# superlinear-ai/raglite

Measured on NVIDIA H100. Metric: queries/sec multi-vector MaxSim over 10M chunks, higher is better.
Workload: dtype f32

## Files before the change

### raglite_b200/csrc/hopper_ptx.cuh

```cuda
#pragma once
#include <cuda.h>
#include <cuda_runtime.h>
#include <stdint.h>

namespace rl {
namespace tc {

__device__ __forceinline__ uint32_t smem_u32(const void* p) { return (uint32_t)__cvta_generic_to_shared(p); }

__device__ __forceinline__ void mbar_init(uint64_t* bar, uint32_t count) {
  asm volatile("mbarrier.init.shared::cta.b64 [%0], %1;" ::"r"(smem_u32(bar)), "r"(count) : "memory");
}
__device__ __forceinline__ void mbar_arrive(uint64_t* bar) {
  asm volatile("mbarrier.arrive.shared::cta.b64 _, [%0];" ::"r"(smem_u32(bar)) : "memory");
}
__device__ __forceinline__ void mbar_arrive_expect_tx(uint64_t* bar, uint32_t bytes) {
  asm volatile("mbarrier.arrive.expect_tx.shared::cta.b64 _, [%0], %1;" ::"r"(smem_u32(bar)), "r"(bytes) : "memory");
}
__device__ __forceinline__ bool mbar_try_wait(uint64_t* bar, uint32_t parity) {
  uint32_t ok;
  asm volatile(
      "{\n\t.reg .pred p;\n\t"
      "mbarrier.try_wait.parity.shared::cta.b64 p, [%1], %2;\n\t"
      "selp.u32 %0, 1, 0, p;\n\t}"
      : "=r"(ok)
      : "r"(smem_u32(bar)), "r"(parity)
      : "memory");
  return ok != 0;
}
__device__ __forceinline__ void mbar_wait(uint64_t* bar, uint32_t parity) {
  if (mbar_try_wait(bar, parity)) return;
  const long long t0 = clock64();
  while (!mbar_try_wait(bar, parity)) {
    if (clock64() - t0 > 20000000000ll) __trap();
  }
}
__device__ __forceinline__ void fence_barrier_init() { asm volatile("fence.mbarrier_init.release.cluster;" ::: "memory"); }
__device__ __forceinline__ void fence_proxy_async() { asm volatile("fence.proxy.async.shared::cta;" ::: "memory"); }

__device__ __forceinline__ void bulk_g2s(void* smem_dst, const void* gsrc, uint32_t bytes, uint64_t* bar) {
  asm volatile("cp.async.bulk.shared::cluster.global.mbarrier::complete_tx::bytes [%0], [%1], %2, [%3];" ::"r"(
                   smem_u32(smem_dst)),
               "l"(gsrc), "r"(bytes), "r"(smem_u32(bar))
               : "memory");
}
__device__ __forceinline__ void tma_load_2d(void* smem_dst, const CUtensorMap* tmap, int c0, int c1, uint64_t* bar) {
  asm volatile(
      "cp.async.bulk.tensor.2d.shared::cluster.global.tile.mbarrier::complete_tx::bytes [%0], [%1, {%3, %4}], [%2];"
      ::"r"(smem_u32(smem_dst)), "l"(tmap), "r"(smem_u32(bar)), "r"(c0), "r"(c1)
      : "memory");
}
__device__ __forceinline__ void tma_prefetch_2d(const CUtensorMap* tmap, int c0, int c1) {
  asm volatile("cp.async.bulk.prefetch.tensor.2d.L2.global.tile [%0, {%1, %2}];" ::"l"(tmap), "r"(c0), "r"(c1) : "memory");
}

__device__ __forceinline__ void prefetch_l2(const void* p) { asm volatile("prefetch.global.L2 [%0];" ::"l"(p)); }
__device__ __forceinline__ float4 ldg_stream(const float* p) {
  float4 v;
  asm volatile("ld.global.nc.L1::no_allocate.v4.f32 {%0, %1, %2, %3}, [%4];"
               : "=f"(v.x), "=f"(v.y), "=f"(v.z), "=f"(v.w)
               : "l"(p));
  return v;
}
__device__ __forceinline__ uint4 ldg_stream_u4(const void* p) {
  uint4 v;
  asm volatile("ld.global.nc.L1::no_allocate.v4.u32 {%0, %1, %2, %3}, [%4];"
               : "=r"(v.x), "=r"(v.y), "=r"(v.z), "=r"(v.w)
               : "l"(p));
  return v;
}

__device__ __forceinline__ void named_bar_sync(int id, int count) {
  asm volatile("bar.sync %0, %1;" ::"r"(id), "r"(count) : "memory");
}

__device__ __forceinline__ uint64_t make_kmajor_sw128_desc(uint32_t smem_addr) {
  return (uint64_t)((smem_addr >> 4) & 0x3FFFu) | (1ull << 16) | (64ull << 32) | (1ull << 62);
}
__device__ __forceinline__ void wgmma_fence() { asm volatile("wgmma.fence.sync.aligned;" ::: "memory"); }
__device__ __forceinline__ void wgmma_commit() { asm volatile("wgmma.commit_group.sync.aligned;" ::: "memory"); }
template <int N>
__device__ __forceinline__ void wgmma_wait() { asm volatile("wgmma.wait_group.sync.aligned %0;" ::"n"(N) : "memory"); }

__device__ __forceinline__ void wgmma_m64n128k16(float (&d)[64], uint64_t a_desc, uint64_t b_desc, uint32_t accumulate) {
  asm volatile(
      "{\n\t.reg .pred p;\n\t"
      "setp.ne.b32 p, %66, 0;\n\t"
      "wgmma.mma_async.sync.aligned.m64n128k16.f32.f16.f16 "
      "{%0, %1, %2, %3, %4, %5, %6, %7, %8, %9, %10, %11, %12, %13, %14, %15, "
      "%16, %17, %18, %19, %20, %21, %22, %23, %24, %25, %26, %27, %28, %29, %30, %31, "
      "%32, %33, %34, %35, %36, %37, %38, %39, %40, %41, %42, %43, %44, %45, %46, %47, "
      "%48, %49, %50, %51, %52, %53, %54, %55, %56, %57, %58, %59, %60, %61, %62, %63}, "
      "%64, %65, p, 1, 1, 0, 0;\n\t}"
      : "+f"(d[0]), "+f"(d[1]), "+f"(d[2]), "+f"(d[3]), "+f"(d[4]), "+f"(d[5]), "+f"(d[6]), "+f"(d[7]),
        "+f"(d[8]), "+f"(d[9]), "+f"(d[10]), "+f"(d[11]), "+f"(d[12]), "+f"(d[13]), "+f"(d[14]), "+f"(d[15]),
        "+f"(d[16]), "+f"(d[17]), "+f"(d[18]), "+f"(d[19]), "+f"(d[20]), "+f"(d[21]), "+f"(d[22]), "+f"(d[23]),
        "+f"(d[24]), "+f"(d[25]), "+f"(d[26]), "+f"(d[27]), "+f"(d[28]), "+f"(d[29]), "+f"(d[30]), "+f"(d[31]),
        "+f"(d[32]), "+f"(d[33]), "+f"(d[34]), "+f"(d[35]), "+f"(d[36]), "+f"(d[37]), "+f"(d[38]), "+f"(d[39]),
        "+f"(d[40]), "+f"(d[41]), "+f"(d[42]), "+f"(d[43]), "+f"(d[44]), "+f"(d[45]), "+f"(d[46]), "+f"(d[47]),
        "+f"(d[48]), "+f"(d[49]), "+f"(d[50]), "+f"(d[51]), "+f"(d[52]), "+f"(d[53]), "+f"(d[54]), "+f"(d[55]),
        "+f"(d[56]), "+f"(d[57]), "+f"(d[58]), "+f"(d[59]), "+f"(d[60]), "+f"(d[61]), "+f"(d[62]), "+f"(d[63])
      : "l"(a_desc), "l"(b_desc), "r"(accumulate)
      : "memory");
}
template <int NACC>
__device__ __forceinline__ void wgmma_slice(float (&d)[NACC], uint64_t a_desc, uint64_t b_desc, bool accumulate) {
  static_assert(NACC == 64 || NACC == 128, "wgmma_slice: N is 128 or 256");
#pragma unroll
  for (int k = 0; k < 4; ++k) {
    const uint32_t acc = (accumulate || k > 0) ? 1u : 0u;
    float(&lo)[64] = *reinterpret_cast<float(*)[64]>(&d[0]);
    wgmma_m64n128k16(lo, a_desc + (uint64_t)(2 * k), b_desc + (uint64_t)(2 * k), acc);
    if constexpr (NACC == 128) {
      float(&hi)[64] = *reinterpret_cast<float(*)[64]>(&d[64]);
      wgmma_m64n128k16(hi, a_desc + (uint64_t)(2 * k), b_desc + (uint64_t)(2 * k + (128 * 128 >> 4)), acc);
    }
  }
}

template <int R>
__device__ __forceinline__ void setmaxnreg_dec() { asm volatile("setmaxnreg.dec.sync.aligned.u32 %0;" ::"n"(R)); }
template <int R>
__device__ __forceinline__ void setmaxnreg_inc() { asm volatile("setmaxnreg.inc.sync.aligned.u32 %0;" ::"n"(R)); }

}
}
```

### raglite_b200/csrc/scan_wgmma.cu

```cuda
#include <cuda.h>
#include <cuda_fp16.h>

#include <cstdlib>
#include <cstring>
#include <type_traits>

#include "hopper_ptx.cuh"
#include "scan_wgmma.cuh"

namespace rl {

namespace {

using namespace tc;

constexpr int kTileM = 128;
constexpr int kSliceK = 64;
constexpr int kNumConsumerWarps = 8;
constexpr int kNumConsumers = kNumConsumerWarps * 32;
constexpr int kFirstLoaderWarp = 8;
constexpr int kNumLoaderWarps = 8;
constexpr int kThreads = (kFirstLoaderWarp + kNumLoaderWarps) * 32;
constexpr int kLoaderRegs = 72;
constexpr int kConsumerRegs = 184;
static_assert(kLoaderRegs + kConsumerRegs == 2 * 65536 / kThreads, "the register split must use exactly the CTA's registers");
constexpr int kMaxStages = 8;
constexpr int kABytes = kTileM * 128;
constexpr uint32_t kSmemBudget = 227 * 1024;
template <int NQ>
__host__ __device__ constexpr int prefetch_items() { return NQ == 128 ? 6 : 0; }
constexpr int kListCap = 1024;
constexpr int kFlushFirst = 192;
constexpr int kFlushAt = 512;
constexpr int kRefreshEvery = 16;
constexpr int kMaxBatchPerLaunch = 1024;

inline int query_group_width(const rl_scan_params* p) {
  const int n_ks = (p->d + kSliceK - 1) / kSliceK;
  return (p->B > 128 && p->e_dtype != 1 && n_ks >= 16) ? 256 : 128;
}

struct TcArgs {
  ScanArgs a;
  const __half* qimg;
  const float* q_scale;
  const float* row_stats;
  int nq;
  int nq_last;
  int par_groups;
  int n_ks;
  int stages;
  int pf_pairs;
};

__device__ __forceinline__ float pow2_scale(float max_abs) {
  return max_abs > 0.f ? exp2f(-ceilf(log2f(max_abs))) : 1.f;
}

struct SmemLayout {
  uint64_t* full;
  uint64_t* empty;
  float* thr;
  float* cs;
  float* thr0;
  float* inv_w;
  uint32_t* hist;
  int* cnt;
  int* basev;
  int* list_n;
  uint32_t* list;
  unsigned char* stage_base;
};

template <int NQ>
__host__ __device__ constexpr uint32_t stage_bytes() { return kABytes + NQ * 128u; }
template <int NQ>
__host__ __device__ constexpr uint32_t tail_bytes() {
  return 2 * kMaxStages * 8 + NQ * (6u * 4u + (uint32_t)kHistBins * 2u) + 16 + kListCap * 12;
}

template <int METRIC, bool EF16, int NQ>
__global__ void __launch_bounds__(kThreads, 1) scan_wgmma_kernel(const __grid_constant__ CUtensorMap tmE, const TcArgs t) {
  extern __shared__ unsigned char smem_dyn[];
  const int P = t.par_groups > 1 ? t.par_groups : 1;
  const int pg = P > 1 ? (int)(blockIdx.x % (unsigned)P) : 0;
  ScanArgs a = t.a;
  const float* q_scale_g = t.q_scale;
  const __half* qimg_g = t.qimg;
  const int nq = (pg == P - 1) ? t.nq_last : t.nq;
  if (P > 1) {
    const int q0p = pg * NQ;
    a.B = min(NQ, t.a.B - q0p);
    a.thr += q0p; a.cand_cnt += q0p; a.eps += q0p; a.hist_inv_w += q0p; a.q_inv_norm += q0p;
    if (a.cnt_all != nullptr) a.cnt_all += q0p;
    a.dump += (size_t)q0p * a.n_sample_rows;
    a.cand += (size_t)q0p * a.cap;
    a.ghist += (size_t)q0p * kHistBins;
    q_scale_g += q0p;
    qimg_g += (size_t)pg * t.n_ks * NQ * kSliceK;
  }
  constexpr uint32_t sbytes = stage_bytes<NQ>();
  SmemLayout s;
  s.full = reinterpret_cast<uint64_t*>(smem_dyn);
  s.empty = s.full + kMaxStages;
  s.thr = reinterpret_cast<float*>(s.empty + kMaxStages);
  s.cs = s.thr + NQ;
  s.thr0 = s.cs + NQ;
  s.inv_w = s.thr0 + NQ;
  s.hist = reinterpret_cast<uint32_t*>(s.inv_w + NQ);
  s.cnt = reinterpret_cast<int*>(s.hist + NQ * kHistBins / 2);
  s.basev = s.cnt + NQ;
  s.list_n = s.basev + NQ;
  s.list = reinterpret_cast<uint32_t*>(s.list_n + 4);
  unsigned char* tail_end = smem_dyn + tail_bytes<NQ>();
  s.stage_base = tail_end + ((1024u - (smem_u32(tail_end) & 1023u)) & 1023u);

  const int warp = threadIdx.x >> 5, lane = threadIdx.x & 31;
  const uint32_t n_tiles = (uint32_t)a.n_mode_blocks;
  const uint32_t first = blockIdx.x / (uint32_t)P;
  const uint32_t stride = gridDim.x / (uint32_t)P;
  const int64_t my_tiles = first < n_tiles ? (n_tiles - first + stride - 1) / stride : 0;
  auto ord_of = [&](int64_t tile) -> uint32_t { return first + (uint32_t)tile * stride; };
  auto block_of = [&](uint32_t ord) -> int64_t {
    const uint32_t S = (uint32_t)a.S;
    return a.dump_mode ? ord * S : (S <= 1u ? ord : ord + ord / (S - 1u) + 1u);
  };
  const uint32_t qbytes = (uint32_t)nq * 128u;
  const unsigned char* qsrc = reinterpret_cast<const unsigned char*>(qimg_g);
  const bool q_thread = threadIdx.x == kFirstLoaderWarp * 32;
  auto put_query = [&](int stage, int ks) {
    mbar_arrive_expect_tx(&s.full[stage], qbytes);
    bulk_g2s(s.stage_base + (size_t)stage * sbytes + kABytes, qsrc + (size_t)ks * qbytes, qbytes, &s.full[stage]);
  };

  if (threadIdx.x == 0) {
    for (int i = 0; i < t.stages; ++i) {
      mbar_init(&s.full[i], (EF16 ? 0 : kNumLoaderWarps) + 1);
      mbar_init(&s.empty[i], kNumConsumerWarps);
    }
    fence_barrier_init();
  }
  for (int i = threadIdx.x; i < NQ; i += blockDim.x) {
    s.thr[i] = (i < a.B && !a.dump_mode) ? a.thr[i] : __int_as_float(0x7f800000);
    s.cs[i] = (i < a.B) ? q_scale_g[i] : 0.f;
    s.cnt[i] = 0;
    s.thr0[i] = s.thr[i];
    s.inv_w[i] = (i < a.B && !a.dump_mode) ? a.hist_inv_w[i] : 0.f;
  }
  for (int i = threadIdx.x; i < NQ * kHistBins / 2; i += blockDim.x) s.hist[i] = 0u;
  if (threadIdx.x == 0) { s.list_n[0] = 0; s.list_n[1] = 0; }
  __syncthreads();
  auto cos_noscale_of = [&]() -> bool {
    return METRIC == RL_METRIC_COSINE &&
           (EF16 || (t.row_stats[2] > 0.f && t.row_stats[2] <= 2.f && t.row_stats[1] <= 1024.f &&
                     t.row_stats[3] == 0.f));
  };

  const bool fast_f32 = !EF16 && a.d % kSliceK == 0 && (t.n_ks & 1) == 0 && a.ld * 64 < (int64_t(1) << 32) &&
                        (METRIC != RL_METRIC_COSINE || cos_noscale_of());
  if (EF16 && warp >= kFirstLoaderWarp) {
    if constexpr (NQ == 256) setmaxnreg_dec<kLoaderRegs>();
    if (q_thread) {
      const int64_t total_items = my_tiles * t.n_ks;
      int ks = 0, stage = 0;
      uint32_t phase = 0;
      int64_t tile = 0;
      auto tile_row0 = [&](int64_t v) -> int { return v < my_tiles ? (int)(block_of(ord_of(v)) * kTileM) : -1; };
      int row0 = tile_row0(0), row0_next = tile_row0(1);
      for (int64_t item = 0; item < total_items; ++item) {
        mbar_wait(&s.empty[stage], phase ^ 1u);
        mbar_arrive_expect_tx(&s.full[stage], qbytes + (uint32_t)kABytes);
        tma_load_2d(s.stage_base + (size_t)stage * sbytes, &tmE, ks * kSliceK, row0, &s.full[stage]);
        bulk_g2s(s.stage_base + (size_t)stage * sbytes + kABytes, qsrc + (size_t)ks * qbytes, qbytes, &s.full[stage]);
        if (row0_next >= 0 && pg == 0) tma_prefetch_2d(&tmE, ks * kSliceK, row0_next);
        if (++ks == t.n_ks) { ks = 0; ++tile; row0 = row0_next; row0_next = tile_row0(tile + 1); }
        if (++stage == t.stages) { stage = 0; phase ^= 1u; }
      }
    }
  } else if (warp >= kFirstLoaderWarp && fast_f32) {
    if constexpr (NQ == 256) setmaxnreg_dec<kLoaderRegs>();
    const int lt = threadIdx.x - kFirstLoaderWarp * 32;
    const int c4 = lt & 15;
    const int r0 = lt >> 4;
    const float gscale = (METRIC == RL_METRIC_COSINE) ? 1.f : pow2_scale(t.row_stats[1]);
    const bool mul = gscale != 1.f;
    uint32_t n_ks = (uint32_t)t.n_ks, n_stages = (uint32_t)t.stages;
    uint32_t pitch16 = (uint32_t)(a.ld * 16 * (int64_t)sizeof(float));
    uint32_t sw_off = (uint32_t)r0 * 128u + ((((uint32_t)c4 >> 1) ^ ((uint32_t)r0 & 7u)) << 4) + (((uint32_t)c4 & 1u) << 3);
    asm volatile("" : "+r"(n_ks), "+r"(n_stages), "+r"(pitch16), "+r"(sw_off));
    const uint32_t total_items = (uint32_t)my_tiles * n_ks;

    struct Cursor { int64_t tile; uint32_t ks; int rows; const unsigned char* ptr; };
    Cursor ld{0, 0u, 0, nullptr};
    auto ld_set_tile = [&]() {
      ld.rows = 0;
      if (ld.tile < my_tiles) {
        const int64_t blk = block_of(ord_of(ld.tile));
        const int64_t rem = a.n_rows - blk * kTileM;
        ld.rows = rem < kTileM ? (int)rem : kTileM;
        ld.ptr = reinterpret_cast<const unsigned char*>(a.E + (size_t)(blk * kTileM + r0) * a.ld + c4 * 4);
      }
    };
    Cursor pf{0, 0u, 0, nullptr};
    auto pf_set_tile = [&]() {
      pf.rows = 0;
      if (pg == 0 && t.pf_pairs > 0 && pf.tile < my_tiles) {
        const int64_t blk = block_of(ord_of(pf.tile));
        const int64_t rem = a.n_rows - blk * kTileM;
        pf.rows = rem < kTileM ? (int)rem : kTileM;
        pf.ptr = reinterpret_cast<const unsigned char*>(a.E + (size_t)(blk * kTileM + (lt >> 1)) * a.ld + (lt & 1) * 32);
        if (METRIC == RL_METRIC_COSINE && lt < 4 && lt * 32 < pf.rows) prefetch_l2(a.inv_norm + blk * kTileM + lt * 32);
      }
    };
    auto pf_pair = [&]() {
      if ((lt >> 1) < pf.rows) { prefetch_l2(pf.ptr); prefetch_l2(pf.ptr + 256); }
      pf.ptr += 512;
      pf.ks += 2;
      if (pf.ks == n_ks) { pf.ks = 0; ++pf.tile; pf_set_tile(); }
    };
    float4 ringA[8], ringB[8];
    auto issue = [&](float4 (&buf)[8], int rows, const unsigned char* src) {
      if (rows == kTileM) {
#pragma unroll
        for (int i = 0; i < 8; ++i) buf[i] = ldg_stream(reinterpret_cast<const float*>(src + (size_t)((uint32_t)i * pitch16)));
      } else {
#pragma unroll
        for (int i = 0; i < 8; ++i) {
          if (r0 + 16 * i < rows) buf[i] = ldg_stream(reinterpret_cast<const float*>(src + (size_t)((uint32_t)i * pitch16)));
          else buf[i] = make_float4(0.f, 0.f, 0.f, 0.f);
        }
      }
    };
    uint32_t stage = 0, phase = 0, st_ks = 0;
    unsigned char* a_dst = s.stage_base + sw_off;
    auto store = [&](const float4 (&buf)[8]) {
      mbar_wait(&s.empty[stage], phase ^ 1u);
      if (q_thread) put_query((int)stage, (int)st_ks);
      if (++st_ks == n_ks) st_ks = 0;
#pragma unroll
      for (int i = 0; i < 8; ++i) {
        float4 v = buf[i];
        if (mul) { v.x *= gscale; v.y *= gscale; v.z *= gscale; v.w *= gscale; }
        const __half2 h01 = __floats2half2_rn(v.x, v.y);
        const __half2 h23 = __floats2half2_rn(v.z, v.w);
        uint2 packed;
        packed.x = *reinterpret_cast<const uint32_t*>(&h01);
        packed.y = *reinterpret_cast<const uint32_t*>(&h23);
        *reinterpret_cast<uint2*>(a_dst + i * 16 * 128) = packed;
      }
      __syncwarp();
      if (lane == 0) mbar_arrive(&s.full[stage]);
      a_dst += sbytes;
      if (++stage == n_stages) { stage = 0; phase ^= 1u; a_dst = s.stage_base + sw_off; }
    };

    ld_set_tile();
    pf_set_tile();
    for (int i = 0; i < t.pf_pairs + 1; ++i) pf_pair();
    if constexpr (NQ == 128) {
      issue(ringA, ld.rows, ld.ptr);
      issue(ringB, ld.rows, ld.ptr + 256);
      for (uint32_t item = 0; item < total_items; item += 2) {
        ld.ptr += 512;
        ld.ks += 2;
        if (ld.ks == n_ks) { ld.ks = 0; ++ld.tile; ld_set_tile(); }
        const int rows = ld.rows;
        const unsigned char* src = ld.ptr;
        store(ringA);
        issue(ringA, rows, src);
        store(ringB);
        issue(ringB, rows, src + 256);
        pf_pair();
      }
    } else {
      issue(ringA, ld.rows, ld.ptr);
      for (uint32_t item = 0; item < total_items; item += 2) {
        const int rows = ld.rows;
        const unsigned char* src = ld.ptr;
        ld.ptr += 512;
        ld.ks += 2;
        if (ld.ks == n_ks) { ld.ks = 0; ++ld.tile; ld_set_tile(); }
        store(ringA);
        issue(ringA, rows, src + 256);
        store(ringA);
        issue(ringA, ld.rows, ld.ptr);
        if constexpr (prefetch_items<NQ>() > 0) pf_pair();
      }
    }
  } else if (warp >= kFirstLoaderWarp) {
    if constexpr (NQ == 256) setmaxnreg_dec<kLoaderRegs>();
    const int lt = threadIdx.x - kFirstLoaderWarp * 32;
    const int c4 = lt & 15;
    const int r0 = lt >> 4;
    const float gscale = (METRIC == RL_METRIC_COSINE) ? 1.f : pow2_scale(t.row_stats[1]);
    const bool noscale = (METRIC == RL_METRIC_COSINE) ? cos_noscale_of() : (gscale == 1.f);
    const uint32_t total_items = (uint32_t)my_tiles * (uint32_t)t.n_ks;
    constexpr int kInFlight = NQ == 128 ? 2 : 1;
    float4 ring[kInFlight][8];
    float rs[8];

    const size_t pitch16_bytes = (size_t)a.ld * 16 * sizeof(float);
    const size_t slice_bytes = kSliceK * sizeof(float);
    int64_t ld_tile = 0;
    int ld_ks = 0, ld_rows = 0;
    const unsigned char* ld_ptr = nullptr;
    auto ld_set_tile = [&]() {
      if (ld_tile < my_tiles) {
        const int64_t blk = block_of(ord_of(ld_tile));
        const int64_t rem = a.n_rows - blk * kTileM;
        ld_rows = rem < kTileM ? (int)rem : kTileM;
        ld_ptr = reinterpret_cast<const unsigned char*>(a.E + (size_t)(blk * kTileM + r0) * a.ld + c4 * 4);
      } else {
        ld_rows = 0;
      }
    };
    int64_t pf_tile = 0;
    int pf_ks = 0, pf_rows = 0;
    const unsigned char* pf_ptr = nullptr;
    auto pf_set_tile = [&]() {
      if (pg == 0 && pf_tile < my_tiles) {
        const int64_t blk = block_of(ord_of(pf_tile));
        const int64_t rem = a.n_rows - blk * kTileM;
        pf_rows = rem < kTileM ? (int)rem : kTileM;
        pf_ptr = reinterpret_cast<const unsigned char*>(a.E + (size_t)(blk * kTileM + (lt >> 1)) * a.ld + (lt & 1) * 32);
        if (METRIC == RL_METRIC_COSINE && lt < 4 && lt * 32 < pf_rows) prefetch_l2(a.inv_norm + blk * kTileM + lt * 32);
      } else {
        pf_rows = 0;
      }
    };
    auto prefetch_item = [&]() {
      if ((lt >> 1) < pf_rows && pf_ks * kSliceK + (lt & 1) * 32 < a.d) prefetch_l2(pf_ptr);
      pf_ptr += slice_bytes;
      if (++pf_ks == t.n_ks) {
        pf_ks = 0;
        ++pf_tile;
        pf_set_tile();
      }
    };
    auto issue_item = [&](float4 (&buf)[8]) {
      const bool col_ok = ld_ks * kSliceK + c4 * 4 < a.d;
      const int rows_left = ld_rows - r0;
      const unsigned char* p = ld_ptr;
      if (col_ok && ld_rows == kTileM) {
#pragma unroll
        for (int i = 0; i < 8; ++i) {
          buf[i] = ldg_stream(reinterpret_cast<const float*>(p));
          p += pitch16_bytes;
        }
      } else {
#pragma unroll
        for (int i = 0; i < 8; ++i) {
          if (col_ok && 16 * i < rows_left) buf[i] = ldg_stream(reinterpret_cast<const float*>(p));
          else buf[i] = make_float4(0.f, 0.f, 0.f, 0.f);
          p += pitch16_bytes;
        }
      }
      ld_ptr += slice_bytes;
      if (++ld_ks == t.n_ks) {
        ld_ks = 0;
        ++ld_tile;
        ld_set_tile();
      }
      if constexpr (prefetch_items<NQ>() > 0) prefetch_item();
    };

    int64_t st_tile = 0;
    int st_ks = 0, stage = 0;
    uint32_t phase = 0;
    auto fetch_scales = [&](int64_t tile) {
#pragma unroll
      for (int i = 0; i < 8; ++i) rs[i] = (METRIC == RL_METRIC_COSINE) ? 0.f : gscale;
      if (METRIC == RL_METRIC_COSINE && !noscale && tile < my_tiles) {
        const int64_t row0 = block_of(ord_of(tile)) * kTileM + r0;
        const int64_t rows_left = a.n_rows - row0;
#pragma unroll
        for (int i = 0; i < 8; ++i) {
          if (16 * i < rows_left) rs[i] = __ldg(a.inv_norm + row0 + 16 * i);
        }
      }
    };
    const uint32_t sw_off = (uint32_t)r0 * 128u + ((((uint32_t)c4 >> 1) ^ ((uint32_t)r0 & 7u)) << 4) + (((uint32_t)c4 & 1u) << 3);
    auto process = [&](float4 (&buf)[8]) {
      mbar_wait(&s.empty[stage], phase ^ 1u);
      if (q_thread) put_query(stage, st_ks);
      unsigned char* A = s.stage_base + (size_t)stage * sbytes + sw_off;
      if (noscale) {
#pragma unroll
        for (int i = 0; i < 8; ++i) {
          const __half2 h01 = __floats2half2_rn(buf[i].x, buf[i].y);
          const __half2 h23 = __floats2half2_rn(buf[i].z, buf[i].w);
          uint2 packed;
          packed.x = *reinterpret_cast<const uint32_t*>(&h01);
          packed.y = *reinterpret_cast<const uint32_t*>(&h23);
          *reinterpret_cast<uint2*>(A + i * 16 * 128) = packed;
        }
      } else {
#pragma unroll
        for (int i = 0; i < 8; ++i) {
          const __half2 h01 = __floats2half2_rn(buf[i].x * rs[i], buf[i].y * rs[i]);
          const __half2 h23 = __floats2half2_rn(buf[i].z * rs[i], buf[i].w * rs[i]);
          uint2 packed;
          packed.x = *reinterpret_cast<const uint32_t*>(&h01);
          packed.y = *reinterpret_cast<const uint32_t*>(&h23);
          *reinterpret_cast<uint2*>(A + i * 16 * 128) = packed;
        }
      }
      __syncwarp();
      if (lane == 0) mbar_arrive(&s.full[stage]);
      issue_item(buf);
      if (++stage == t.stages) { stage = 0; phase ^= 1u; }
      if (++st_ks == t.n_ks) { st_ks = 0; ++st_tile; fetch_scales(st_tile); }
    };

    fetch_scales(0);
    ld_set_tile();
    pf_set_tile();
    for (int i = 0; i < prefetch_items<NQ>(); ++i) prefetch_item();
    for (int i = 0; i < kInFlight; ++i) issue_item(ring[i]);
    for (uint32_t item = 0; item < total_items; item += kInFlight) {
      process(ring[0]);
      if constexpr (kInFlight == 2) {
        if (item + 1 < total_items) process(ring[1]);
      }
    }
  } else {
    if constexpr (NQ == 256) setmaxnreg_inc<kConsumerRegs>();
    const int wg = warp >> 2;
    const int r_lo = wg * 64 + (warp & 3) * 16 + (lane >> 2);
    const int c_lane = 2 * (lane & 3);
    const int et = threadIdx.x;
    bool flushed_once = false;
    int stage = 0;
    uint32_t phase = 0;
    float acc[NQ / 2];
    const bool cos_noscale = cos_noscale_of();
    for (int64_t tile = 0; tile < my_tiles; ++tile) {
      int prev = -1;
      for (int ks = 0; ks < t.n_ks; ++ks) {
        mbar_wait(&s.full[stage], phase);
        fence_proxy_async();
        const uint32_t st_addr = smem_u32(s.stage_base + (size_t)stage * sbytes);
        wgmma_fence();
        wgmma_slice(acc, make_kmajor_sw128_desc(st_addr + (uint32_t)wg * (64u * 128u)), make_kmajor_sw128_desc(st_addr + kABytes),
                    ks > 0);
        wgmma_commit();
        if (prev >= 0) {
          wgmma_wait<1>();
          __syncwarp();
          if (lane == 0) mbar_arrive(&s.empty[prev]);
        }
        prev = stage;
        if (++stage == t.stages) { stage = 0; phase ^= 1u; }
      }
      wgmma_wait<0>();
      __syncwarp();
      if (lane == 0) mbar_arrive(&s.empty[prev]);

      const int64_t ord = ord_of(tile);
      const int64_t blk = block_of(ord);
      int r_in[2];
      int64_t row[2];
      bool valid[2], masked_alive[2];
      float bias[2], lane_scale[2];
#pragma unroll
      for (int h = 0; h < 2; ++h) {
        r_in[h] = r_lo + 8 * h;
        row[h] = blk * kTileM + r_in[h];
        valid[h] = row[h] < a.n_rows;
        masked_alive[h] = false;
        if (valid[h] && a.row_allowed != nullptr) {
          valid[h] = a.row_allowed[row[h]] != 0;
          if (!valid[h] && a.cnt_all != nullptr) masked_alive[h] = a.row_alive == nullptr || a.row_alive[row[h]] != 0;
        }
        bias[h] = (METRIC == RL_METRIC_L2 && valid[h]) ? -a.sq_norm[row[h]] : 0.f;
        lane_scale[h] = (METRIC == RL_METRIC_COSINE && cos_noscale && valid[h]) ? __ldg(a.inv_norm + row[h]) : 1.f;
      }
      auto key_of = [&](float accv, int h, float cs) -> float {
        return METRIC != RL_METRIC_COSINE ? fmaf(accv, cs, bias[h]) : accv * lane_scale[h];
      };
      if (a.dump_mode) {
#pragma unroll
        for (int c8 = 0; c8 < NQ / 8; ++c8) {
#pragma unroll
          for (int e = 0; e < 4; ++e) {
            const int h = e >> 1, col = 8 * c8 + c_lane + (e & 1);
            if (col < a.B) {
              const float key = key_of(acc[4 * c8 + e], h, s.cs[col]);
              a.dump[(size_t)col * a.n_sample_rows + ord * kTileM + r_in[h]] = valid[h] ? key : kNegInf;
            }
          }
        }
      } else {
#pragma unroll
        for (int c8 = 0; c8 < NQ / 8; ++c8) {
          if (8 * c8 >= nq) break;
          const int c = 8 * c8 + c_lane;
          const float2 th = *reinterpret_cast<const float2*>(s.thr + c);
          const float2 sc = METRIC != RL_METRIC_COSINE ? *reinterpret_cast<const float2*>(s.cs + c) : make_float2(0.f, 0.f);
#pragma unroll
          for (int e = 0; e < 4; ++e) {
            const int h = e >> 1, col = c + (e & 1);
            const float key = key_of(acc[4 * c8 + e], h, (e & 1) ? sc.y : sc.x);
            if (key >= ((e & 1) ? th.y : th.x)) {
              if (masked_alive[h]) atomicAdd(a.cnt_all + col, 1);
              if (valid[h]) {
                const int pos = atomicAdd(&s.list_n[0], 1);
                const int hb = col * kHistBins + hist_bin(key, s.thr0[col], s.inv_w[col]);
                atomicAdd(&s.hist[hb >> 1], 1u << ((hb & 1) * 16));
                if (pos < kListCap) {
                  s.list[pos * 3 + 0] = (uint32_t)col;
                  s.list[pos * 3 + 1] = __float_as_uint(key);
                  s.list[pos * 3 + 2] = (uint32_t)row[h];
                } else {
                  emit_candidate(a, col, key, (int32_t)row[h]);
                }
              }
            }
          }
        }
        named_bar_sync(1, kNumConsumers);
        const int n_all = s.list_n[0];
        named_bar_sync(1, kNumConsumers);
        const bool last = tile + 1 == my_tiles;
        const bool do_flush = n_all >= (flushed_once ? kFlushAt : kFlushFirst) || (last && n_all > 0);
        if (do_flush) {
          flushed_once = true;
          const int n = min(n_all, kListCap);
          for (int e = et; e < n; e += kNumConsumers) {
            const int col = (int)s.list[e * 3 + 0];
            s.list[e * 3 + 0] = (uint32_t)col | ((uint32_t)atomicAdd(&s.cnt[col], 1) << 16);
          }
          named_bar_sync(1, kNumConsumers);
          for (int col = et; col < NQ; col += kNumConsumers) {
            const int c = s.cnt[col];
            if (c > 0) {
              s.basev[col] = atomicAdd(a.cand_cnt + col, c);
              s.cnt[col] = 0;
            }
          }
          for (int w = et; w < NQ * kHistBins / 2; w += kNumConsumers) {
            const uint32_t h = s.hist[w];
            if (h != 0u) {
              if (h & 0xFFFFu) atomicAdd(a.ghist + 2 * w, (int)(h & 0xFFFFu));
              if (h >> 16) atomicAdd(a.ghist + 2 * w + 1, (int)(h >> 16));
              s.hist[w] = 0u;
            }
          }
          named_bar_sync(1, kNumConsumers);
          if (et == 0) s.list_n[0] = 0;
          for (int e = et; e < n; e += kNumConsumers) {
            const uint32_t w0 = s.list[e * 3 + 0];
            const int col = (int)(w0 & 0xFFFFu);
            const int slot = s.basev[col] + (int)(w0 >> 16);
            if (slot < a.cap)
              a.cand[(size_t)col * a.cap + slot] = Cand{__uint_as_float(s.list[e * 3 + 1]), (int32_t)s.list[e * 3 + 2]};
          }
        }
        const bool periodic = (tile % kRefreshEvery) == kRefreshEvery - 1;
        if ((do_flush || periodic) && !last) {
          for (int col = et; col < a.B; col += kNumConsumers) {
            const int4* gh = reinterpret_cast<const int4*>(a.ghist + (size_t)col * kHistBins);
            int cnts[kHistBins];
#pragma unroll
            for (int q4 = 0; q4 < kHistBins / 4; ++q4) {
              const int4 v4 = __ldcg(gh + q4);
              cnts[4 * q4] = v4.x; cnts[4 * q4 + 1] = v4.y; cnts[4 * q4 + 2] = v4.z; cnts[4 * q4 + 3] = v4.w;
            }
            int cum = 0, best = -1;
#pragma unroll
            for (int bb = kHistBins - 1; bb >= 1; --bb) {
              cum += cnts[bb];
              if (best < 0 && cum >= a.sel_count) best = bb;
            }
            if (best >= 1 && s.inv_w[col] > 0.f) {
              const float nt = s.thr0[col] + (float)best / s.inv_w[col] - 2.f * a.eps[col];
              if (nt > s.thr[col]) s.thr[col] = nt;
            }
          }
        }
        if (do_flush || periodic) named_bar_sync(1, kNumConsumers);
      }
    }
  }
}

__global__ void __launch_bounds__(128) query_image_kernel(const float* __restrict__ Q, int B, int d, int metric,
                                                          const float* __restrict__ q_inv_norm,
                                                          const float* __restrict__ row_stats, float* __restrict__ q_scale,
                                                          __half* __restrict__ qimg, int n_ks, int rows_scaled, int gw) {
  __shared__ float red[4];
  const int b = blockIdx.x;
  const int group = b / gw, n = b % gw;
  const int nq = min(gw, (B - group * gw + 15) / 16 * 16);
  const float* q = Q + (size_t)b * d;
  float scale;
  if (metric == RL_METRIC_COSINE) {
    scale = q_inv_norm[b];
    if (threadIdx.x == 0) q_scale[b] = 1.f;
  } else {
    float m = 0.f;
    for (int c = threadIdx.x; c < d; c += blockDim.x) m = fmaxf(m, fabsf(q[c]));
#pragma unroll
    for (int o = 16; o > 0; o >>= 1) m = fmaxf(m, __shfl_xor_sync(0xffffffffu, m, o));
    if ((threadIdx.x & 31) == 0) red[threadIdx.x >> 5] = m;
    __syncthreads();
    m = fmaxf(fmaxf(red[0], red[1]), fmaxf(red[2], red[3]));
    scale = pow2_scale(m);
    const float rs_e = rows_scaled ? pow2_scale(row_stats[1]) : 1.f;
    if (threadIdx.x == 0) q_scale[b] = (metric == RL_METRIC_L2 ? 2.f : 1.f) / (scale * rs_e);
  }
  __half* img = qimg + (size_t)group * n_ks * gw * kSliceK;
  for (int c = threadIdx.x; c < n_ks * kSliceK; c += blockDim.x) {
    const int ks = c / kSliceK, e = c % kSliceK;
    const float v = c < d ? q[c] * scale : 0.f;
    const int chunk = e >> 3, within = e & 7;
    const size_t off = ((size_t)ks * nq + n) * kSliceK + (size_t)(((chunk ^ (n & 7)) << 3) + within);
    img[off] = __float2half_rn(v);
  }
}

typedef CUresult (*ScanEncodeTiledFn)(CUtensorMap*, CUtensorMapDataType, cuuint32_t, void*, const cuuint64_t*, const cuuint64_t*,
                                      const cuuint32_t*, const cuuint32_t*, CUtensorMapInterleave, CUtensorMapSwizzle,
                                      CUtensorMapL2promotion, CUtensorMapFloatOOBfill);
ScanEncodeTiledFn scan_encode_tiled_fn() {
  static ScanEncodeTiledFn fn = []() -> ScanEncodeTiledFn {
    void* p = nullptr;
    cudaDriverEntryPointQueryResult q;
    if (cudaGetDriverEntryPoint("cuTensorMapEncodeTiled", &p, cudaEnableDefault, &q) != cudaSuccess || q != cudaDriverEntryPointSuccess)
      return nullptr;
    return reinterpret_cast<ScanEncodeTiledFn>(p);
  }();
  return fn;
}
bool make_corpus_tensor_map(CUtensorMap* tm, const void* E, int64_t n_rows, int64_t ld, int d) {
  ScanEncodeTiledFn enc = scan_encode_tiled_fn();
  if (enc == nullptr || (reinterpret_cast<uintptr_t>(E) & 15) != 0 || (ld * 2) % 16 != 0 || n_rows >= (int64_t(1) << 31)) return false;
  const cuuint64_t gdim[2] = {(cuuint64_t)d, (cuuint64_t)n_rows};
  const cuuint64_t gstr[1] = {(cuuint64_t)ld * sizeof(__half)};
  const cuuint32_t box[2] = {(cuuint32_t)kSliceK, (cuuint32_t)kTileM};
  const cuuint32_t estr[2] = {1, 1};
  return enc(tm, CU_TENSOR_MAP_DATA_TYPE_FLOAT16, 2, const_cast<void*>(E), gdim, gstr, box, estr, CU_TENSOR_MAP_INTERLEAVE_NONE,
             CU_TENSOR_MAP_SWIZZLE_128B, CU_TENSOR_MAP_L2_PROMOTION_L2_128B, CU_TENSOR_MAP_FLOAT_OOB_FILL_NONE) == CUDA_SUCCESS;
}

}

bool wgmma_scan_supported(const rl_scan_params* p) {
  if (p == nullptr || p->n_rows <= 0 || p->B <= 0) return false;
  if (p->e_dtype == 1 && (p->d % 8 != 0 || p->ld % 8 != 0)) return false;
  if (p->d % 4 != 0 || p->ld % 4 != 0) return false;
  if ((reinterpret_cast<uintptr_t>(p->E) & 15) != 0) return false;
  if ((p->d + kSliceK - 1) / kSliceK > 1024) return false;
  return true;
}

size_t wgmma_qimg_bytes(const rl_scan_params* p) {
  const int n_ks = (p->d + kSliceK - 1) / kSliceK;
  const int gw = query_group_width(p);
  const int groups = (p->B + gw - 1) / gw;
  return (size_t)groups * n_ks * gw * kSliceK * sizeof(__half);
}

int wgmma_prepare_queries(const rl_scan_params* p, const float* q_inv_norm, float* q_scale, void* qimg, cudaStream_t stream) {
  const int n_ks = (p->d + kSliceK - 1) / kSliceK;
  RL_CUDA_CHECK(cudaMemsetAsync(qimg, 0, wgmma_qimg_bytes(p), stream));
  query_image_kernel<<<p->B, 128, 0, stream>>>(p->Q, p->B, p->d, p->metric, q_inv_norm, p->row_stats, q_scale,
                                                 reinterpret_cast<__half*>(qimg), n_ks, p->e_dtype == 1 ? 0 : 1,
                                                 query_group_width(p));
  RL_CUDA_CHECK(cudaGetLastError());
  return RL_OK;
}

namespace {

template <int NQ>
int launch_scan_groups(const ScanArgs& a_in, const rl_scan_params* p, const float* q_scale, const void* qimg, int sm_count,
                       const CUtensorMap& tmE, cudaStream_t stream) {
  const int n_ks = (p->d + kSliceK - 1) / kSliceK;
  const int groups = (a_in.B + NQ - 1) / NQ;
  int max_groups = sm_count / 2;
  if (max_groups > kMaxBatchPerLaunch / NQ) max_groups = kMaxBatchPerLaunch / NQ;
  if (max_groups < 1) max_groups = 1;
  for (int g0 = 0; g0 < groups; g0 += max_groups) {
    TcArgs t;
    t.a = a_in;
    const int q0 = g0 * NQ;
    const int ng = groups - g0 < max_groups ? groups - g0 : max_groups;
    const int nb = a_in.B - q0 < ng * NQ ? a_in.B - q0 : ng * NQ;
    t.a.B = nb;
    t.a.thr = a_in.thr + q0;
    t.a.dump = a_in.dump + (size_t)q0 * a_in.n_sample_rows;
    t.a.cand = a_in.cand + (size_t)q0 * a_in.cap;
    t.a.cand_cnt = a_in.cand_cnt + q0;
    t.a.ghist = a_in.ghist + (size_t)q0 * kHistBins;
    t.a.eps = a_in.eps + q0;
    t.a.hist_inv_w = a_in.hist_inv_w + q0;
    t.a.q_inv_norm = a_in.q_inv_norm + q0;
    t.a.cnt_all = a_in.cnt_all ? a_in.cnt_all + q0 : nullptr;
    t.qimg = reinterpret_cast<const __half*>(qimg) + (size_t)g0 * n_ks * NQ * kSliceK;
    t.q_scale = q_scale + q0;
    t.row_stats = p->row_stats;
    t.par_groups = ng;
    const int last_b = nb - (ng - 1) * NQ;
    t.nq_last = (last_b + 15) / 16 * 16;
    t.nq = ng > 1 ? NQ : t.nq_last;
    t.n_ks = n_ks;
    t.pf_pairs = prefetch_items<NQ>() / 2;
    const uint32_t avail = kSmemBudget - 1024 - tail_bytes<NQ>();
    int stages = (int)(avail / stage_bytes<NQ>());
    if (stages > kMaxStages) stages = kMaxStages;
    RL_REQUIRE(stages >= 2, RL_EUNSUPPORTED, "tensor-core scan: not enough shared memory for 2 stages");
    t.stages = stages;
    const size_t smem = (size_t)stages * stage_bytes<NQ>() + tail_bytes<NQ>() + 1024;
    auto launch = [&](auto kernel) -> int {
      RL_CUDA_CHECK(cudaFuncSetAttribute(kernel, cudaFuncAttributeMaxDynamicSharedMemorySize, (int)smem));
      const int lanes = sm_count / t.par_groups;
      const unsigned grid = (unsigned)((a_in.n_mode_blocks < lanes ? a_in.n_mode_blocks : lanes) * t.par_groups);
      kernel<<<grid, kThreads, smem, stream>>>(tmE, t);
      RL_CUDA_CHECK(cudaGetLastError());
      return RL_OK;
    };
    int rc;
    if (p->e_dtype == 1) {
      if constexpr (NQ == 128) {
        if (p->metric == RL_METRIC_COSINE) rc = launch(scan_wgmma_kernel<RL_METRIC_COSINE, true, NQ>);
        else if (p->metric == RL_METRIC_DOT) rc = launch(scan_wgmma_kernel<RL_METRIC_DOT, true, NQ>);
        else rc = launch(scan_wgmma_kernel<RL_METRIC_L2, true, NQ>);
      } else {
        RL_REQUIRE(false, RL_EUNSUPPORTED, "tensor-core scan: fp16 storage runs query groups of 128");
      }
    } else {
      if (p->metric == RL_METRIC_COSINE) rc = launch(scan_wgmma_kernel<RL_METRIC_COSINE, false, NQ>);
      else if (p->metric == RL_METRIC_DOT) rc = launch(scan_wgmma_kernel<RL_METRIC_DOT, false, NQ>);
      else rc = launch(scan_wgmma_kernel<RL_METRIC_L2, false, NQ>);
    }
    if (rc != RL_OK) return rc;
  }
  return RL_OK;
}

}

int launch_scan_wgmma(const ScanArgs& a_in, const rl_scan_params* p, const float* q_scale, const void* qimg, int sm_count,
                      cudaStream_t stream) {
  if (a_in.n_mode_blocks == 0 || a_in.B == 0) return RL_OK;
  RL_REQUIRE(p->row_stats != nullptr, RL_EINVAL, "tensor-core scan needs row_stats");
  CUtensorMap tmE;
  memset(&tmE, 0, sizeof(tmE));
  RL_REQUIRE(p->e_dtype != 1 || make_corpus_tensor_map(&tmE, p->E, p->n_rows, p->ld, p->d), RL_EUNSUPPORTED,
             "fp16 storage: no TMA tensor map for the corpus (cuTensorMapEncodeTiled unavailable or failed)");
  if (query_group_width(p) == 256) return launch_scan_groups<256>(a_in, p, q_scale, qimg, sm_count, tmE, stream);
  return launch_scan_groups<128>(a_in, p, q_scale, qimg, sm_count, tmE, stream);
}

}
```

Measured before the change: 763.5.

## Load f32 corpus via TMA and convert to fp16 in consumer registers for RS wgmma

Replaces the eight loader warps that read f32 corpus rows with ld.global, converted them to fp16 and stored swizzled tiles, with a single TMA producer thread. That thread loads raw f32 boxes with an L2 evict-first hint into separate corpus and query ring buffers. Consumers now read the f32 fragments from shared memory, scale and convert them to fp16 in registers, and feed them to register-sourced wgmma. This removes the loader warps' global-load and smem-store traffic and gives consumers more registers. In exchange, consumers take on the conversion work, and each f32 corpus slot uses twice the shared memory, so fewer ring slots fit.

```diff
diff --git a/raglite_b200/csrc/hopper_ptx.cuh b/raglite_b200/csrc/hopper_ptx.cuh
--- a/raglite_b200/csrc/hopper_ptx.cuh
+++ b/raglite_b200/csrc/hopper_ptx.cuh
@@ -36,7 +36,6 @@
   }
 }
 __device__ __forceinline__ void fence_barrier_init() { asm volatile("fence.mbarrier_init.release.cluster;" ::: "memory"); }
-__device__ __forceinline__ void fence_proxy_async() { asm volatile("fence.proxy.async.shared::cta;" ::: "memory"); }
 
 __device__ __forceinline__ void bulk_g2s(void* smem_dst, const void* gsrc, uint32_t bytes, uint64_t* bar) {
   asm volatile("cp.async.bulk.shared::cluster.global.mbarrier::complete_tx::bytes [%0], [%1], %2, [%3];" ::"r"(
@@ -50,24 +49,16 @@
       ::"r"(smem_u32(smem_dst)), "l"(tmap), "r"(smem_u32(bar)), "r"(c0), "r"(c1)
       : "memory");
 }
+__device__ __forceinline__ void tma_load_2d_evict_first(void* smem_dst, const CUtensorMap* tmap, int c0, int c1, uint64_t* bar) {
+  asm volatile(
+      "{\n\t.reg .b64 pol;\n\t"
+      "createpolicy.fractional.L2::evict_first.b64 pol, 1.0;\n\t"
+      "cp.async.bulk.tensor.2d.shared::cluster.global.tile.mbarrier::complete_tx::bytes.L2::cache_hint [%0], [%1, {%3, %4}], [%2], pol;\n\t}"
+      ::"r"(smem_u32(smem_dst)), "l"(tmap), "r"(smem_u32(bar)), "r"(c0), "r"(c1)
+      : "memory");
+}
 __device__ __forceinline__ void tma_prefetch_2d(const CUtensorMap* tmap, int c0, int c1) {
   asm volatile("cp.async.bulk.prefetch.tensor.2d.L2.global.tile [%0, {%1, %2}];" ::"l"(tmap), "r"(c0), "r"(c1) : "memory");
-}
-
-__device__ __forceinline__ void prefetch_l2(const void* p) { asm volatile("prefetch.global.L2 [%0];" ::"l"(p)); }
-__device__ __forceinline__ float4 ldg_stream(const float* p) {
-  float4 v;
-  asm volatile("ld.global.nc.L1::no_allocate.v4.f32 {%0, %1, %2, %3}, [%4];"
-               : "=f"(v.x), "=f"(v.y), "=f"(v.z), "=f"(v.w)
-               : "l"(p));
-  return v;
-}
-__device__ __forceinline__ uint4 ldg_stream_u4(const void* p) {
-  uint4 v;
-  asm volatile("ld.global.nc.L1::no_allocate.v4.u32 {%0, %1, %2, %3}, [%4];"
-               : "=r"(v.x), "=r"(v.y), "=r"(v.z), "=r"(v.w)
-               : "l"(p));
-  return v;
 }
 
 __device__ __forceinline__ void named_bar_sync(int id, int count) {
@@ -103,6 +94,27 @@
       : "l"(a_desc), "l"(b_desc), "r"(accumulate)
       : "memory");
 }
+__device__ __forceinline__ void wgmma_m64n128k16_rs(float (&d)[64], const uint32_t (&a)[4], uint64_t b_desc, uint32_t accumulate) {
+  asm volatile(
+      "{\n\t.reg .pred p;\n\t"
+      "setp.ne.b32 p, %69, 0;\n\t"
+      "wgmma.mma_async.sync.aligned.m64n128k16.f32.f16.f16 "
+      "{%0, %1, %2, %3, %4, %5, %6, %7, %8, %9, %10, %11, %12, %13, %14, %15, "
+      "%16, %17, %18, %19, %20, %21, %22, %23, %24, %25, %26, %27, %28, %29, %30, %31, "
+      "%32, %33, %34, %35, %36, %37, %38, %39, %40, %41, %42, %43, %44, %45, %46, %47, "
+      "%48, %49, %50, %51, %52, %53, %54, %55, %56, %57, %58, %59, %60, %61, %62, %63}, "
+      "{%64, %65, %66, %67}, %68, p, 1, 1, 0;\n\t}"
+      : "+f"(d[0]), "+f"(d[1]), "+f"(d[2]), "+f"(d[3]), "+f"(d[4]), "+f"(d[5]), "+f"(d[6]), "+f"(d[7]),
+        "+f"(d[8]), "+f"(d[9]), "+f"(d[10]), "+f"(d[11]), "+f"(d[12]), "+f"(d[13]), "+f"(d[14]), "+f"(d[15]),
+        "+f"(d[16]), "+f"(d[17]), "+f"(d[18]), "+f"(d[19]), "+f"(d[20]), "+f"(d[21]), "+f"(d[22]), "+f"(d[23]),
+        "+f"(d[24]), "+f"(d[25]), "+f"(d[26]), "+f"(d[27]), "+f"(d[28]), "+f"(d[29]), "+f"(d[30]), "+f"(d[31]),
+        "+f"(d[32]), "+f"(d[33]), "+f"(d[34]), "+f"(d[35]), "+f"(d[36]), "+f"(d[37]), "+f"(d[38]), "+f"(d[39]),
+        "+f"(d[40]), "+f"(d[41]), "+f"(d[42]), "+f"(d[43]), "+f"(d[44]), "+f"(d[45]), "+f"(d[46]), "+f"(d[47]),
+        "+f"(d[48]), "+f"(d[49]), "+f"(d[50]), "+f"(d[51]), "+f"(d[52]), "+f"(d[53]), "+f"(d[54]), "+f"(d[55]),
+        "+f"(d[56]), "+f"(d[57]), "+f"(d[58]), "+f"(d[59]), "+f"(d[60]), "+f"(d[61]), "+f"(d[62]), "+f"(d[63])
+      : "r"(a[0]), "r"(a[1]), "r"(a[2]), "r"(a[3]), "l"(b_desc), "r"(accumulate)
+      : "memory");
+}
 template <int NACC>
 __device__ __forceinline__ void wgmma_slice(float (&d)[NACC], uint64_t a_desc, uint64_t b_desc, bool accumulate) {
   static_assert(NACC == 64 || NACC == 128, "wgmma_slice: N is 128 or 256");
@@ -117,6 +129,21 @@
     }
   }
 }
+template <int NACC>
+__device__ __forceinline__ void wgmma_slice_rs(float (&d)[NACC], const uint32_t (&a)[16], uint64_t b_desc, bool accumulate) {
+  static_assert(NACC == 64 || NACC == 128, "wgmma_slice_rs: N is 128 or 256");
+#pragma unroll
+  for (int k = 0; k < 4; ++k) {
+    const uint32_t acc = (accumulate || k > 0) ? 1u : 0u;
+    const uint32_t(&ak)[4] = *reinterpret_cast<const uint32_t(*)[4]>(&a[4 * k]);
+    float(&lo)[64] = *reinterpret_cast<float(*)[64]>(&d[0]);
+    wgmma_m64n128k16_rs(lo, ak, b_desc + (uint64_t)(2 * k), acc);
+    if constexpr (NACC == 128) {
+      float(&hi)[64] = *reinterpret_cast<float(*)[64]>(&d[64]);
+      wgmma_m64n128k16_rs(hi, ak, b_desc + (uint64_t)(2 * k + (128 * 128 >> 4)), acc);
+    }
+  }
+}
 
 template <int R>
 __device__ __forceinline__ void setmaxnreg_dec() { asm volatile("setmaxnreg.dec.sync.aligned.u32 %0;" ::"n"(R)); }
diff --git a/raglite_b200/csrc/scan_wgmma.cu b/raglite_b200/csrc/scan_wgmma.cu
--- a/raglite_b200/csrc/scan_wgmma.cu
+++ b/raglite_b200/csrc/scan_wgmma.cu
@@ -18,17 +18,15 @@
 constexpr int kSliceK = 64;
 constexpr int kNumConsumerWarps = 8;
 constexpr int kNumConsumers = kNumConsumerWarps * 32;
-constexpr int kFirstLoaderWarp = 8;
-constexpr int kNumLoaderWarps = 8;
-constexpr int kThreads = (kFirstLoaderWarp + kNumLoaderWarps) * 32;
-constexpr int kLoaderRegs = 72;
-constexpr int kConsumerRegs = 184;
-static_assert(kLoaderRegs + kConsumerRegs == 2 * 65536 / kThreads, "the register split must use exactly the CTA's registers");
-constexpr int kMaxStages = 8;
-constexpr int kABytes = kTileM * 128;
+constexpr int kProducerWarp = 8;
+constexpr int kThreads = (kProducerWarp + 4) * 32;
+constexpr int kProducerRegs = 40;
+constexpr int kConsumerRegs = 232;
+static_assert(128 * kProducerRegs + kNumConsumers * kConsumerRegs <= 65536, "the register split must fit the register file");
+constexpr int kMaxSlots = 8;
+constexpr int kF16SliceBytes = kTileM * 128;
+constexpr int kF32BoxBytes = kTileM * 128;
 constexpr uint32_t kSmemBudget = 227 * 1024;
-template <int NQ>
-__host__ __device__ constexpr int prefetch_items() { return NQ == 128 ? 6 : 0; }
 constexpr int kListCap = 1024;
 constexpr int kFlushFirst = 192;
 constexpr int kFlushAt = 512;
@@ -49,8 +47,8 @@
   int nq_last;
   int par_groups;
   int n_ks;
-  int stages;
-  int pf_pairs;
+  int c_slots;
+  int q_slots;
 };
 
 __device__ __forceinline__ float pow2_scale(float max_abs) {
@@ -58,8 +56,10 @@
 }
 
 struct SmemLayout {
-  uint64_t* full;
-  uint64_t* empty;
+  uint64_t* c_full;
+  uint64_t* c_empty;
+  uint64_t* q_full;
+  uint64_t* q_empty;
   float* thr;
   float* cs;
   float* thr0;
@@ -69,14 +69,16 @@
   int* basev;
   int* list_n;
   uint32_t* list;
-  unsigned char* stage_base;
+  unsigned char* c_base;
+  unsigned char* q_base;
 };
 
+__host__ __device__ constexpr uint32_t corpus_slot_bytes(bool ef16) { return ef16 ? kF16SliceBytes : 2u * kF32BoxBytes; }
 template <int NQ>
-__host__ __device__ constexpr uint32_t stage_bytes() { return kABytes + NQ * 128u; }
+__host__ __device__ constexpr uint32_t query_slot_bytes() { return NQ * 128u; }
 template <int NQ>
 __host__ __device__ constexpr uint32_t tail_bytes() {
-  return 2 * kMaxStages * 8 + NQ * (6u * 4u + (uint32_t)kHistBins * 2u) + 16 + kListCap * 12;
+  return 4 * kMaxSlots * 8 + NQ * (6u * 4u + (uint32_t)kHistBins * 2u) + 16 + kListCap * 12;
 }
 
 template <int METRIC, bool EF16, int NQ>
@@ -99,11 +101,14 @@
     q_scale_g += q0p;
     qimg_g += (size_t)pg * t.n_ks * NQ * kSliceK;
   }
-  constexpr uint32_t sbytes = stage_bytes<NQ>();
+  constexpr uint32_t cbytes = corpus_slot_bytes(EF16);
+  constexpr uint32_t qslot = query_slot_bytes<NQ>();
   SmemLayout s;
-  s.full = reinterpret_cast<uint64_t*>(smem_dyn);
-  s.empty = s.full + kMaxStages;
-  s.thr = reinterpret_cast<float*>(s.empty + kMaxStages);
+  s.c_full = reinterpret_cast<uint64_t*>(smem_dyn);
+  s.c_empty = s.c_full + kMaxSlots;
+  s.q_full = s.c_empty + kMaxSlots;
+  s.q_empty = s.q_full + kMaxSlots;
+  s.thr = reinterpret_cast<float*>(s.q_empty + kMaxSlots);
   s.cs = s.thr + NQ;
   s.thr0 = s.cs + NQ;
   s.inv_w = s.thr0 + NQ;
@@ -113,7 +118,8 @@
   s.list_n = s.basev + NQ;
   s.list = reinterpret_cast<uint32_t*>(s.list_n + 4);
   unsigned char* tail_end = smem_dyn + tail_bytes<NQ>();
-  s.stage_base = tail_end + ((1024u - (smem_u32(tail_end) & 1023u)) & 1023u);
+  s.c_base = tail_end + ((1024u - (smem_u32(tail_end) & 1023u)) & 1023u);
+  s.q_base = s.c_base + (size_t)t.c_slots * cbytes;
 
   const int warp = threadIdx.x >> 5, lane = threadIdx.x & 31;
   const uint32_t n_tiles = (uint32_t)a.n_mode_blocks;
@@ -126,17 +132,15 @@
     return a.dump_mode ? ord * S : (S <= 1u ? ord : ord + ord / (S - 1u) + 1u);
   };
   const uint32_t qbytes = (uint32_t)nq * 128u;
-  const unsigned char* qsrc = reinterpret_cast<const unsigned char*>(qimg_g);
-  const bool q_thread = threadIdx.x == kFirstLoaderWarp * 32;
-  auto put_query = [&](int stage, int ks) {
-    mbar_arrive_expect_tx(&s.full[stage], qbytes);
-    bulk_g2s(s.stage_base + (size_t)stage * sbytes + kABytes, qsrc + (size_t)ks * qbytes, qbytes, &s.full[stage]);
-  };
 
   if (threadIdx.x == 0) {
-    for (int i = 0; i < t.stages; ++i) {
-      mbar_init(&s.full[i], (EF16 ? 0 : kNumLoaderWarps) + 1);
-      mbar_init(&s.empty[i], kNumConsumerWarps);
+    for (int i = 0; i < t.c_slots; ++i) {
+      mbar_init(&s.c_full[i], 1);
+      mbar_init(&s.c_empty[i], kNumConsumerWarps);
+    }
+    for (int i = 0; i < t.q_slots; ++i) {
+      mbar_init(&s.q_full[i], 1);
+      mbar_init(&s.q_empty[i], kNumConsumerWarps);
     }
     fence_barrier_init();
   }
@@ -150,314 +154,151 @@
   for (int i = threadIdx.x; i < NQ * kHistBins / 2; i += blockDim.x) s.hist[i] = 0u;
   if (threadIdx.x == 0) { s.list_n[0] = 0; s.list_n[1] = 0; }
   __syncthreads();
-  auto cos_noscale_of = [&]() -> bool {
-    return METRIC == RL_METRIC_COSINE &&
-           (EF16 || (t.row_stats[2] > 0.f && t.row_stats[2] <= 2.f && t.row_stats[1] <= 1024.f &&
-                     t.row_stats[3] == 0.f));
-  };
-
-  const bool fast_f32 = !EF16 && a.d % kSliceK == 0 && (t.n_ks & 1) == 0 && a.ld * 64 < (int64_t(1) << 32) &&
-                        (METRIC != RL_METRIC_COSINE || cos_noscale_of());
-  if (EF16 && warp >= kFirstLoaderWarp) {
-    if constexpr (NQ == 256) setmaxnreg_dec<kLoaderRegs>();
-    if (q_thread) {
-      const int64_t total_items = my_tiles * t.n_ks;
-      int ks = 0, stage = 0;
-      uint32_t phase = 0;
+
+  if (warp >= kProducerWarp) {
+    setmaxnreg_dec<kProducerRegs>();
+    const uint32_t total_items = (uint32_t)my_tiles * (uint32_t)t.n_ks;
+    if (threadIdx.x == kProducerWarp * 32) {
+      uint32_t slot = 0, phase = 0, ks = 0;
       int64_t tile = 0;
       auto tile_row0 = [&](int64_t v) -> int { return v < my_tiles ? (int)(block_of(ord_of(v)) * kTileM) : -1; };
       int row0 = tile_row0(0), row0_next = tile_row0(1);
-      for (int64_t item = 0; item < total_items; ++item) {
-        mbar_wait(&s.empty[stage], phase ^ 1u);
-        mbar_arrive_expect_tx(&s.full[stage], qbytes + (uint32_t)kABytes);
-        tma_load_2d(s.stage_base + (size_t)stage * sbytes, &tmE, ks * kSliceK, row0, &s.full[stage]);
-        bulk_g2s(s.stage_base + (size_t)stage * sbytes + kABytes, qsrc + (size_t)ks * qbytes, qbytes, &s.full[stage]);
-        if (row0_next >= 0 && pg == 0) tma_prefetch_2d(&tmE, ks * kSliceK, row0_next);
-        if (++ks == t.n_ks) { ks = 0; ++tile; row0 = row0_next; row0_next = tile_row0(tile + 1); }
-        if (++stage == t.stages) { stage = 0; phase ^= 1u; }
+      for (uint32_t item = 0; item < total_items; ++item) {
+        mbar_wait(&s.c_empty[slot], phase ^ 1u);
+        unsigned char* dst = s.c_base + (size_t)slot * cbytes;
+        mbar_arrive_expect_tx(&s.c_full[slot], cbytes);
+        if constexpr (EF16) {
+          tma_load_2d(dst, &tmE, (int)ks * kSliceK, row0, &s.c_full[slot]);
+          if (row0_next >= 0 && pg == 0) tma_prefetch_2d(&tmE, (int)ks * kSliceK, row0_next);
+        } else {
+          tma_load_2d_evict_first(dst, &tmE, (int)ks * kSliceK, row0, &s.c_full[slot]);
+          tma_load_2d_evict_first(dst + kF32BoxBytes, &tmE, (int)ks * kSliceK + kSliceK / 2, row0, &s.c_full[slot]);
+        }
+        if (++ks == (uint32_t)t.n_ks) { ks = 0; ++tile; row0 = row0_next; row0_next = tile_row0(tile + 1); }
+        if (++slot == (uint32_t)t.c_slots) { slot = 0; phase ^= 1u; }
       }
-    }
-  } else if (warp >= kFirstLoaderWarp && fast_f32) {
-    if constexpr (NQ == 256) setmaxnreg_dec<kLoaderRegs>();
-    const int lt = threadIdx.x - kFirstLoaderWarp * 32;
-    const int c4 = lt & 15;
-    const int r0 = lt >> 4;
-    const float gscale = (METRIC == RL_METRIC_COSINE) ? 1.f : pow2_scale(t.row_stats[1]);
-    const bool mul = gscale != 1.f;
-    uint32_t n_ks = (uint32_t)t.n_ks, n_stages = (uint32_t)t.stages;
-    uint32_t pitch16 = (uint32_t)(a.ld * 16 * (int64_t)sizeof(float));
-    uint32_t sw_off = (uint32_t)r0 * 128u + ((((uint32_t)c4 >> 1) ^ ((uint32_t)r0 & 7u)) << 4) + (((uint32_t)c4 & 1u) << 3);
-    asm volatile("" : "+r"(n_ks), "+r"(n_stages), "+r"(pitch16), "+r"(sw_off));
-    const uint32_t total_items = (uint32_t)my_tiles * n_ks;
-
-    struct Cursor { int64_t tile; uint32_t ks; int rows; const unsigned char* ptr; };
-    Cursor ld{0, 0u, 0, nullptr};
-    auto ld_set_tile = [&]() {
-      ld.rows = 0;
-      if (ld.tile < my_tiles) {
-        const int64_t blk = block_of(ord_of(ld.tile));
-        const int64_t rem = a.n_rows - blk * kTileM;
-        ld.rows = rem < kTileM ? (int)rem : kTileM;
-        ld.ptr = reinterpret_cast<const unsigned char*>(a.E + (size_t)(blk * kTileM + r0) * a.ld + c4 * 4);
-      }
-    };
-    Cursor pf{0, 0u, 0, nullptr};
-    auto pf_set_tile = [&]() {
-      pf.rows = 0;
-      if (pg == 0 && t.pf_pairs > 0 && pf.tile < my_tiles) {
-        const int64_t blk = block_of(ord_of(pf.tile));
-        const int64_t rem = a.n_rows - blk * kTileM;
-        pf.rows = rem < kTileM ? (int)rem : kTileM;
-        pf.ptr = reinterpret_cast<const unsigned char*>(a.E + (size_t)(blk * kTileM + (lt >> 1)) * a.ld + (lt & 1) * 32);
-        if (METRIC == RL_METRIC_COSINE && lt < 4 && lt * 32 < pf.rows) prefetch_l2(a.inv_norm + blk * kTileM + lt * 32);
-      }
-    };
-    auto pf_pair = [&]() {
-      if ((lt >> 1) < pf.rows) { prefetch_l2(pf.ptr); prefetch_l2(pf.ptr + 256); }
-      pf.ptr += 512;
-      pf.ks += 2;
-      if (pf.ks == n_ks) { pf.ks = 0; ++pf.tile; pf_set_tile(); }
-    };
-    float4 ringA[8], ringB[8];
-    auto issue = [&](float4 (&buf)[8], int rows, const unsigned char* src) {
-      if (rows == kTileM) {
-#pragma unroll
-        for (int i = 0; i < 8; ++i) buf[i] = ldg_stream(reinterpret_cast<const float*>(src + (size_t)((uint32_t)i * pitch16)));
-      } else {
-#pragma unroll
-        for (int i = 0; i < 8; ++i) {
-          if (r0 + 16 * i < rows) buf[i] = ldg_stream(reinterpret_cast<const float*>(src + (size_t)((uint32_t)i * pitch16)));
-          else buf[i] = make_float4(0.f, 0.f, 0.f, 0.f);
-        }
-      }
-    };
-    uint32_t stage = 0, phase = 0, st_ks = 0;
-    unsigned char* a_dst = s.stage_base + sw_off;
-    auto store = [&](const float4 (&buf)[8]) {
-      mbar_wait(&s.empty[stage], phase ^ 1u);
-      if (q_thread) put_query((int)stage, (int)st_ks);
-      if (++st_ks == n_ks) st_ks = 0;
-#pragma unroll
-      for (int i = 0; i < 8; ++i) {
-        float4 v = buf[i];
-        if (mul) { v.x *= gscale; v.y *= gscale; v.z *= gscale; v.w *= gscale; }
-        const __half2 h01 = __floats2half2_rn(v.x, v.y);
-        const __half2 h23 = __floats2half2_rn(v.z, v.w);
-        uint2 packed;
-        packed.x = *reinterpret_cast<const uint32_t*>(&h01);
-        packed.y = *reinterpret_cast<const uint32_t*>(&h23);
-        *reinterpret_cast<uint2*>(a_dst + i * 16 * 128) = packed;
-      }
-      __syncwarp();
-      if (lane == 0) mbar_arrive(&s.full[stage]);
-      a_dst += sbytes;
-      if (++stage == n_stages) { stage = 0; phase ^= 1u; a_dst = s.stage_base + sw_off; }
-    };
-
-    ld_set_tile();
-    pf_set_tile();
-    for (int i = 0; i < t.pf_pairs + 1; ++i) pf_pair();
-    if constexpr (NQ == 128) {
-      issue(ringA, ld.rows, ld.ptr);
-      issue(ringB, ld.rows, ld.ptr + 256);
-      for (uint32_t item = 0; item < total_items; item += 2) {
-        ld.ptr += 512;
-        ld.ks += 2;
-        if (ld.ks == n_ks) { ld.ks = 0; ++ld.tile; ld_set_tile(); }
-        const int rows = ld.rows;
-        const unsigned char* src = ld.ptr;
-        store(ringA);
-        issue(ringA, rows, src);
-        store(ringB);
-        issue(ringB, rows, src + 256);
-        pf_pair();
-      }
-    } else {
-      issue(ringA, ld.rows, ld.ptr);
-      for (uint32_t item = 0; item < total_items; item += 2) {
-        const int rows = ld.rows;
-        const unsigned char* src = ld.ptr;
-        ld.ptr += 512;
-        ld.ks += 2;
-        if (ld.ks == n_ks) { ld.ks = 0; ++ld.tile; ld_set_tile(); }
-        store(ringA);
-        issue(ringA, rows, src + 256);
-        store(ringA);
-        issue(ringA, ld.rows, ld.ptr);
-        if constexpr (prefetch_items<NQ>() > 0) pf_pair();
-      }
-    }
-  } else if (warp >= kFirstLoaderWarp) {
-    if constexpr (NQ == 256) setmaxnreg_dec<kLoaderRegs>();
-    const int lt = threadIdx.x - kFirstLoaderWarp * 32;
-    const int c4 = lt & 15;
-    const int r0 = lt >> 4;
-    const float gscale = (METRIC == RL_METRIC_COSINE) ? 1.f : pow2_scale(t.row_stats[1]);
-    const bool noscale = (METRIC == RL_METRIC_COSINE) ? cos_noscale_of() : (gscale == 1.f);
-    const uint32_t total_items = (uint32_t)my_tiles * (uint32_t)t.n_ks;
-    constexpr int kInFlight = NQ == 128 ? 2 : 1;
-    float4 ring[kInFlight][8];
-    float rs[8];
-
-    const size_t pitch16_bytes = (size_t)a.ld * 16 * sizeof(float);
-    const size_t slice_bytes = kSliceK * sizeof(float);
-    int64_t ld_tile = 0;
-    int ld_ks = 0, ld_rows = 0;
-    const unsigned char* ld_ptr = nullptr;
-    auto ld_set_tile = [&]() {
-      if (ld_tile < my_tiles) {
-        const int64_t blk = block_of(ord_of(ld_tile));
-        const int64_t rem = a.n_rows - blk * kTileM;
-        ld_rows = rem < kTileM ? (int)rem : kTileM;
-        ld_ptr = reinterpret_cast<const unsigned char*>(a.E + (size_t)(blk * kTileM + r0) * a.ld + c4 * 4);
-      } else {
-        ld_rows = 0;
-      }
-    };
-    int64_t pf_tile = 0;
-    int pf_ks = 0, pf_rows = 0;
-    const unsigned char* pf_ptr = nullptr;
-    auto pf_set_tile = [&]() {
-      if (pg == 0 && pf_tile < my_tiles) {
-        const int64_t blk = block_of(ord_of(pf_tile));
-        const int64_t rem = a.n_rows - blk * kTileM;
-        pf_rows = rem < kTileM ? (int)rem : kTileM;
-        pf_ptr = reinterpret_cast<const unsigned char*>(a.E + (size_t)(blk * kTileM + (lt >> 1)) * a.ld + (lt & 1) * 32);
-        if (METRIC == RL_METRIC_COSINE && lt < 4 && lt * 32 < pf_rows) prefetch_l2(a.inv_norm + blk * kTileM + lt * 32);
-      } else {
-        pf_rows = 0;
-      }
-    };
-    auto prefetch_item = [&]() {
-      if ((lt >> 1) < pf_rows && pf_ks * kSliceK + (lt & 1) * 32 < a.d) prefetch_l2(pf_ptr);
-      pf_ptr += slice_bytes;
-      if (++pf_ks == t.n_ks) {
-        pf_ks = 0;
-        ++pf_tile;
-        pf_set_tile();
-      }
-    };
-    auto issue_item = [&](float4 (&buf)[8]) {
-      const bool col_ok = ld_ks * kSliceK + c4 * 4 < a.d;
-      const int rows_left = ld_rows - r0;
-      const unsigned char* p = ld_ptr;
-      if (col_ok && ld_rows == kTileM) {
-#pragma unroll
-        for (int i = 0; i < 8; ++i) {
-          buf[i] = ldg_stream(reinterpret_cast<const float*>(p));
-          p += pitch16_bytes;
-        }
-      } else {
-#pragma unroll
-        for (int i = 0; i < 8; ++i) {
-          if (col_ok && 16 * i < rows_left) buf[i] = ldg_stream(reinterpret_cast<const float*>(p));
-          else buf[i] = make_float4(0.f, 0.f, 0.f, 0.f);
-          p += pitch16_bytes;
-        }
-      }
-      ld_ptr += slice_bytes;
-      if (++ld_ks == t.n_ks) {
-        ld_ks = 0;
-        ++ld_tile;
-        ld_set_tile();
-      }
-      if constexpr (prefetch_items<NQ>() > 0) prefetch_item();
-    };
-
-    int64_t st_tile = 0;
-    int st_ks = 0, stage = 0;
-    uint32_t phase = 0;
-    auto fetch_scales = [&](int64_t tile) {
-#pragma unroll
-      for (int i = 0; i < 8; ++i) rs[i] = (METRIC == RL_METRIC_COSINE) ? 0.f : gscale;
-      if (METRIC == RL_METRIC_COSINE && !noscale && tile < my_tiles) {
-        const int64_t row0 = block_of(ord_of(tile)) * kTileM + r0;
-        const int64_t rows_left = a.n_rows - row0;
-#pragma unroll
-        for (int i = 0; i < 8; ++i) {
-          if (16 * i < rows_left) rs[i] = __ldg(a.inv_norm + row0 + 16 * i);
-        }
-      }
-    };
-    const uint32_t sw_off = (uint32_t)r0 * 128u + ((((uint32_t)c4 >> 1) ^ ((uint32_t)r0 & 7u)) << 4) + (((uint32_t)c4 & 1u) << 3);
-    auto process = [&](float4 (&buf)[8]) {
-      mbar_wait(&s.empty[stage], phase ^ 1u);
-      if (q_thread) put_query(stage, st_ks);
-      unsigned char* A = s.stage_base + (size_t)stage * sbytes + sw_off;
-      if (noscale) {
-#pragma unroll
-        for (int i = 0; i < 8; ++i) {
-          const __half2 h01 = __floats2half2_rn(buf[i].x, buf[i].y);
-          const __half2 h23 = __floats2half2_rn(buf[i].z, buf[i].w);
-          uint2 packed;
-          packed.x = *reinterpret_cast<const uint32_t*>(&h01);
-          packed.y = *reinterpret_cast<const uint32_t*>(&h23);
-          *reinterpret_cast<uint2*>(A + i * 16 * 128) = packed;
-        }
-      } else {
-#pragma unroll
-        for (int i = 0; i < 8; ++i) {
-          const __half2 h01 = __floats2half2_rn(buf[i].x * rs[i], buf[i].y * rs[i]);
-          const __half2 h23 = __floats2half2_rn(buf[i].z * rs[i], buf[i].w * rs[i]);
-          uint2 packed;
-          packed.x = *reinterpret_cast<const uint32_t*>(&h01);
-          packed.y = *reinterpret_cast<const uint32_t*>(&h23);
-          *reinterpret_cast<uint2*>(A + i * 16 * 128) = packed;
-        }
-      }
-      __syncwarp();
-      if (lane == 0) mbar_arrive(&s.full[stage]);
-      issue_item(buf);
-      if (++stage == t.stages) { stage = 0; phase ^= 1u; }
-      if (++st_ks == t.n_ks) { st_ks = 0; ++st_tile; fetch_scales(st_tile); }
-    };
-
-    fetch_scales(0);
-    ld_set_tile();
-    pf_set_tile();
-    for (int i = 0; i < prefetch_items<NQ>(); ++i) prefetch_item();
-    for (int i = 0; i < kInFlight; ++i) issue_item(ring[i]);
-    for (uint32_t item = 0; item < total_items; item += kInFlight) {
-      process(ring[0]);
-      if constexpr (kInFlight == 2) {
-        if (item + 1 < total_items) process(ring[1]);
+    } else if (threadIdx.x == (kProducerWarp + 1) * 32) {
+      const unsigned char* qsrc = reinterpret_cast<const unsigned char*>(qimg_g);
+      uint32_t slot = 0, phase = 0, ks = 0;
+      for (uint32_t item = 0; item < total_items; ++item) {
+        mbar_wait(&s.q_empty[slot], phase ^ 1u);
+        mbar_arrive_expect_tx(&s.q_full[slot], qbytes);
+        bulk_g2s(s.q_base + (size_t)slot * qslot, qsrc + (size_t)ks * qbytes, qbytes, &s.q_full[slot]);
+        if (++ks == (uint32_t)t.n_ks) ks = 0;
+        if (++slot == (uint32_t)t.q_slots) { slot = 0; phase ^= 1u; }
       }
     }
   } else {
-    if constexpr (NQ == 256) setmaxnreg_inc<kConsumerRegs>();
+    setmaxnreg_inc<kConsumerRegs>();
     const int wg = warp >> 2;
     const int r_lo = wg * 64 + (warp & 3) * 16 + (lane >> 2);
     const int c_lane = 2 * (lane & 3);
     const int et = threadIdx.x;
     bool flushed_once = false;
-    int stage = 0;
-    uint32_t phase = 0;
+    uint32_t c_slot = 0, c_phase = 0, q_slot = 0, q_phase = 0;
     float acc[NQ / 2];
-    const bool cos_noscale = cos_noscale_of();
+    const bool cos_noscale =
+        METRIC == RL_METRIC_COSINE && (EF16 || (t.row_stats[2] > 0.f && t.row_stats[2] <= 2.f && t.row_stats[1] <= 1024.f &&
+                                                t.row_stats[3] == 0.f));
+    const float gscale = (METRIC == RL_METRIC_COSINE) ? 1.f : pow2_scale(t.row_stats[1]);
+    const bool scaled = !EF16 && ((METRIC == RL_METRIC_COSINE) ? !cos_noscale : gscale != 1.f);
+    uint32_t frag_off[4];
+#pragma unroll
+    for (int jh = 0; jh < 4; ++jh)
+      frag_off[jh] = (uint32_t)r_lo * 128u + ((((uint32_t)jh * 2u + (uint32_t)((lane & 3) >> 1)) ^ (uint32_t)((lane >> 2) & 7)) << 4) +
+                     (uint32_t)(lane & 1) * 8u;
+    const uint32_t q_base_u32 = smem_u32(s.q_base);
     for (int64_t tile = 0; tile < my_tiles; ++tile) {
-      int prev = -1;
-      for (int ks = 0; ks < t.n_ks; ++ks) {
-        mbar_wait(&s.full[stage], phase);
-        fence_proxy_async();
-        const uint32_t st_addr = smem_u32(s.stage_base + (size_t)stage * sbytes);
-        wgmma_fence();
-        wgmma_slice(acc, make_kmajor_sw128_desc(st_addr + (uint32_t)wg * (64u * 128u)), make_kmajor_sw128_desc(st_addr + kABytes),
-                    ks > 0);
-        wgmma_commit();
-        if (prev >= 0) {
-          wgmma_wait<1>();
-          __syncwarp();
-          if (lane == 0) mbar_arrive(&s.empty[prev]);
-        }
-        prev = stage;
-        if (++stage == t.stages) { stage = 0; phase ^= 1u; }
-      }
-      wgmma_wait<0>();
-      __syncwarp();
-      if (lane == 0) mbar_arrive(&s.empty[prev]);
-
       const int64_t ord = ord_of(tile);
       const int64_t blk = block_of(ord);
+      float inv[2] = {0.f, 0.f};
+      if (METRIC == RL_METRIC_COSINE) {
+#pragma unroll
+        for (int h = 0; h < 2; ++h) {
+          const int64_t r = blk * kTileM + r_lo + 8 * h;
+          if (r < a.n_rows) inv[h] = __ldg(a.inv_norm + r);
+        }
+      }
+      const float rs0 = METRIC == RL_METRIC_COSINE ? inv[0] : gscale;
+      const float rs1 = METRIC == RL_METRIC_COSINE ? inv[1] : gscale;
+      int prev_q = -1;
+      if constexpr (EF16) {
+        int prev_c = -1;
+        for (int ks = 0; ks < t.n_ks; ++ks) {
+          mbar_wait(&s.c_full[c_slot], c_phase);
+          mbar_wait(&s.q_full[q_slot], q_phase);
+          const uint32_t a_addr = smem_u32(s.c_base + (size_t)c_slot * cbytes) + (uint32_t)wg * (64u * 128u);
+          wgmma_fence();
+          wgmma_slice(acc, make_kmajor_sw128_desc(a_addr), make_kmajor_sw128_desc(q_base_u32 + q_slot * qslot), ks > 0);
+          wgmma_commit();
+          if (prev_q >= 0) {
+            wgmma_wait<1>();
+            __syncwarp();
+            if (lane == 0) { mbar_arrive(&s.c_empty[prev_c]); mbar_arrive(&s.q_empty[prev_q]); }
+          }
+          prev_c = (int)c_slot;
+          prev_q = (int)q_slot;
+          if (++c_slot == (uint32_t)t.c_slots) { c_slot = 0; c_phase ^= 1u; }
+          if (++q_slot == (uint32_t)t.q_slots) { q_slot = 0; q_phase ^= 1u; }
+        }
+        wgmma_wait<0>();
+        __syncwarp();
+        if (lane == 0) { mbar_arrive(&s.c_empty[prev_c]); mbar_arrive(&s.q_empty[prev_q]); }
+      } else {
+        auto load_convert = [&](uint32_t (&f)[16]) {
+          mbar_wait(&s.c_full[c_slot], c_phase);
+          const unsigned char* src = s.c_base + (size_t)c_slot * cbytes;
+          float2 v[16];
+#pragma unroll
+          for (int j = 0; j < 4; ++j) {
+#pragma unroll
+            for (int i = 0; i < 4; ++i) {
+              const uint32_t off = (uint32_t)(j >> 1) * kF32BoxBytes + frag_off[2 * (j & 1) + (i >> 1)] + (uint32_t)(i & 1) * 1024u;
+              v[4 * j + i] = *reinterpret_cast<const float2*>(src + off);
+            }
+          }
+          if (scaled) {
+#pragma unroll
+            for (int i = 0; i < 16; ++i) {
+              const float r = (i & 1) ? rs1 : rs0;
+              v[i].x *= r;
+              v[i].y *= r;
+            }
+          }
+#pragma unroll
+          for (int i = 0; i < 16; ++i) {
+            const __half2 h = __floats2half2_rn(v[i].x, v[i].y);
+            f[i] = *reinterpret_cast<const uint32_t*>(&h);
+          }
+          __syncwarp();
+          if (lane == 0) mbar_arrive(&s.c_empty[c_slot]);
+          if (++c_slot == (uint32_t)t.c_slots) { c_slot = 0; c_phase ^= 1u; }
+        };
+        auto mma_step = [&](uint32_t (&f)[16], uint32_t (&f_next)[16], int ks) {
+          mbar_wait(&s.q_full[q_slot], q_phase);
+          wgmma_fence();
+          wgmma_slice_rs(acc, f, make_kmajor_sw128_desc(q_base_u32 + q_slot * qslot), ks > 0);
+          wgmma_commit();
+          if (prev_q >= 0) {
+            wgmma_wait<1>();
+            __syncwarp();
+            if (lane == 0) mbar_arrive(&s.q_empty[prev_q]);
+          }
+          prev_q = (int)q_slot;
+          if (++q_slot == (uint32_t)t.q_slots) { q_slot = 0; q_phase ^= 1u; }
+          if (ks + 1 < t.n_ks) load_convert(f_next);
+        };
+        uint32_t fa[16], fb[16];
+        load_convert(fa);
+        for (int ks = 0; ks < t.n_ks; ks += 2) {
+          mma_step(fa, fb, ks);
+          if (ks + 1 < t.n_ks) mma_step(fb, fa, ks + 1);
+        }
+        wgmma_wait<0>();
+        __syncwarp();
+        if (lane == 0) mbar_arrive(&s.q_empty[prev_q]);
+      }
+
       int r_in[2];
       int64_t row[2];
       bool valid[2], masked_alive[2];
@@ -473,7 +314,7 @@
           if (!valid[h] && a.cnt_all != nullptr) masked_alive[h] = a.row_alive == nullptr || a.row_alive[row[h]] != 0;
         }
         bias[h] = (METRIC == RL_METRIC_L2 && valid[h]) ? -a.sq_norm[row[h]] : 0.f;
-        lane_scale[h] = (METRIC == RL_METRIC_COSINE && cos_noscale && valid[h]) ? __ldg(a.inv_norm + row[h]) : 1.f;
+        lane_scale[h] = (METRIC == RL_METRIC_COSINE && cos_noscale && valid[h]) ? inv[h] : 1.f;
       }
       auto key_of = [&](float accv, int h, float cs) -> float {
         return METRIC != RL_METRIC_COSINE ? fmaf(accv, cs, bias[h]) : accv * lane_scale[h];
@@ -632,15 +473,19 @@
   }();
   return fn;
 }
-bool make_corpus_tensor_map(CUtensorMap* tm, const void* E, int64_t n_rows, int64_t ld, int d) {
+bool make_corpus_tensor_map(CUtensorMap* tm, const void* E, bool fp16, int64_t n_rows, int64_t ld, int d) {
   ScanEncodeTiledFn enc = scan_encode_tiled_fn();
-  if (enc == nullptr || (reinterpret_cast<uintptr_t>(E) & 15) != 0 || (ld * 2) % 16 != 0 || n_rows >= (int64_t(1) << 31)) return false;
+  const int64_t esize = fp16 ? 2 : 4;
+  if (enc == nullptr || (reinterpret_cast<uintptr_t>(E) & 15) != 0 || (ld * esize) % 16 != 0 || n_rows >= (int64_t(1) << 31))
+    return false;
   const cuuint64_t gdim[2] = {(cuuint64_t)d, (cuuint64_t)n_rows};
-  const cuuint64_t gstr[1] = {(cuuint64_t)ld * sizeof(__half)};
-  const cuuint32_t box[2] = {(cuuint32_t)kSliceK, (cuuint32_t)kTileM};
+  const cuuint64_t gstr[1] = {(cuuint64_t)(ld * esize)};
+  const cuuint32_t box[2] = {(cuuint32_t)(128 / esize), (cuuint32_t)kTileM};
   const cuuint32_t estr[2] = {1, 1};
-  return enc(tm, CU_TENSOR_MAP_DATA_TYPE_FLOAT16, 2, const_cast<void*>(E), gdim, gstr, box, estr, CU_TENSOR_MAP_INTERLEAVE_NONE,
-             CU_TENSOR_MAP_SWIZZLE_128B, CU_TENSOR_MAP_L2_PROMOTION_L2_128B, CU_TENSOR_MAP_FLOAT_OOB_FILL_NONE) == CUDA_SUCCESS;
+  const CUtensorMapL2promotion promo = fp16 ? CU_TENSOR_MAP_L2_PROMOTION_L2_128B : CU_TENSOR_MAP_L2_PROMOTION_L2_256B;
+  return enc(tm, fp16 ? CU_TENSOR_MAP_DATA_TYPE_FLOAT16 : CU_TENSOR_MAP_DATA_TYPE_FLOAT32, 2, const_cast<void*>(E), gdim, gstr,
+             box, estr, CU_TENSOR_MAP_INTERLEAVE_NONE, CU_TENSOR_MAP_SWIZZLE_128B, promo, CU_TENSOR_MAP_FLOAT_OOB_FILL_NONE) ==
+         CUDA_SUCCESS;
 }
 
 }
@@ -705,13 +550,14 @@
     t.nq_last = (last_b + 15) / 16 * 16;
     t.nq = ng > 1 ? NQ : t.nq_last;
     t.n_ks = n_ks;
-    t.pf_pairs = prefetch_items<NQ>() / 2;
+    const uint32_t cb = corpus_slot_bytes(p->e_dtype == 1), qb = query_slot_bytes<NQ>();
     const uint32_t avail = kSmemBudget - 1024 - tail_bytes<NQ>();
-    int stages = (int)(avail / stage_bytes<NQ>());
-    if (stages > kMaxStages) stages = kMaxStages;
-    RL_REQUIRE(stages >= 2, RL_EUNSUPPORTED, "tensor-core scan: not enough shared memory for 2 stages");
-    t.stages = stages;
-    const size_t smem = (size_t)stages * stage_bytes<NQ>() + tail_bytes<NQ>() + 1024;
+    int slots = (int)(avail / (cb + qb));
+    if (slots > kMaxSlots) slots = kMaxSlots;
+    RL_REQUIRE(slots >= 2, RL_EUNSUPPORTED, "tensor-core scan: not enough shared memory for 2 ring slots");
+    t.c_slots = slots;
+    t.q_slots = slots;
+    const size_t smem = (size_t)t.c_slots * cb + (size_t)t.q_slots * qb + tail_bytes<NQ>() + 1024;
     auto launch = [&](auto kernel) -> int {
       RL_CUDA_CHECK(cudaFuncSetAttribute(kernel, cudaFuncAttributeMaxDynamicSharedMemorySize, (int)smem));
       const int lanes = sm_count / t.par_groups;
@@ -747,8 +593,8 @@
   RL_REQUIRE(p->row_stats != nullptr, RL_EINVAL, "tensor-core scan needs row_stats");
   CUtensorMap tmE;
   memset(&tmE, 0, sizeof(tmE));
-  RL_REQUIRE(p->e_dtype != 1 || make_corpus_tensor_map(&tmE, p->E, p->n_rows, p->ld, p->d), RL_EUNSUPPORTED,
-             "fp16 storage: no TMA tensor map for the corpus (cuTensorMapEncodeTiled unavailable or failed)");
+  RL_REQUIRE(make_corpus_tensor_map(&tmE, p->E, p->e_dtype == 1, p->n_rows, p->ld, p->d), RL_EUNSUPPORTED,
+             "tensor-core scan: no TMA tensor map for the corpus (cuTensorMapEncodeTiled unavailable or failed)");
   if (query_group_width(p) == 256) return launch_scan_groups<256>(a_in, p, q_scale, qimg, sm_count, tmE, stream);
   return launch_scan_groups<128>(a_in, p, q_scale, qimg, sm_count, tmE, stream);
 }
```

After: 778.2, median of 6. 1.9% higher.
